# OxygenLost/dddmr_navigation

Hardware: AMD Instinct MI355X
Metric: scored trajectories/sec (N_traj x N_steps) (higher is better)
Workload: dtype f32; 1 GPU; C3: 16384 trajectories x 80 steps vs 500000-point cloud, 80-pose prune plan, shipped critic stack; scene_layout=r02, trajectories_per_gpu=16384, steps_per_trajectory=80, parallelism=single, contexts_per_gpu=1

## Files before the change

dddmr_navigation_amd/csrc/rollout_engine.hip:

```cpp
#include <hip/hip_runtime.h>
#include <dlfcn.h>
#include <rccl/rccl.h>

#include <algorithm>
#include <atomic>
#include <cmath>
#include <cstdarg>
#include <chrono>
#include <cstdio>
#include <cstdlib>
#include <cstring>
#include <memory>
#include <mutex>
#include <string>
#include <vector>

#include "rollout_kernels.hip.h"
#include "tick_plan.hip.h"
#include "perception_kernels.hip.h"
#include "depth_feed.hip.h"
#include "depth_image.hip.h"
#include "depth_clear.hip.h"
#include "lidar_sweep.hip.h"
#include "lidar_features.hip.h"
// ... 6 lines not shown

constexpr int kCloudBufs = 3;

struct MarkingState;
struct DepthMarkState;
struct DepthLayerState;
struct StackState;
struct MclState;
template <class T>
using ModuleSlot = std::unique_ptr<T, LateDelete<T>>;

struct SourceOwned {
  std::unique_ptr<PerceptionScratch> feed;
  std::unique_ptr<DepthSource> depth;
  std::unique_ptr<DepthImage> dimg;
  std::unique_ptr<LidarSweep> sweep;
  Owned scan_obs;
  float4* obs = nullptr;
  DcFrustum frustum{};
};

}

struct dddmr_rollout_ctx {
  dddmr_rollout_config cfg{};
  std::vector<dddmr_theory_config> theories;
  int device = 0;
  hipStream_t stream = nullptr, copy_stream = nullptr;
  DevAllocs mem;
  HostAllocs host;
  TrajInfo* traj_info = nullptr;
  double2* st_sc = nullptr;
  float2* st_xy = nullptr;
  size_t st_cap = 0;
  hipEvent_t ev0 = nullptr, ev1 = nullptr, evs0 = nullptr, evs1 = nullptr, cloud_ready[kCloudBufs] = {nullptr, nullptr, nullptr};

  float4* cloud_dev[kCloudBufs] = {nullptr, nullptr, nullptr};
  uint32_t cloud_n[kCloudBufs] = {0, 0, 0};
  SourceLayout cloud_layout[kCloudBufs];
  uint2* pt_slot = nullptr;
  Pt3* sorted = nullptr;
  uint32_t *cell_count = nullptr, *cell_start = nullptr;
  uint32_t* row_tab = nullptr;
  float* axes_dev = nullptr;
  float4* samples_dev = nullptr;
  float4* plan_dev = nullptr;
  float* plan_pairs_dev = nullptr;
  double* costs = nullptr;
  TrajPartial* partial = nullptr;
  int32_t* steps = nullptr;
  float4* samples_out = nullptr;
  int64_t* best_key = nullptr;
  uint32_t* overflow = nullptr;
  DevResult* result_dev = nullptr;
  uint32_t* tickets = nullptr;
  float4* blocked_plan = nullptr;
  uint32_t* blocked_flags = nullptr;
  uint32_t* traj_load = nullptr;
  uint32_t* assign = nullptr;
  TickFeedback feedback;
  TickKnobs knobs;
  bool poison = false;
  bool host_prof = false;
  bool debug_grid = false;
  int ceil_blocks = 0;
  double prof_ns[4] = {0, 0, 0, 0};
// ... 492 lines not shown

void set_no_winner(dddmr_rollout_result* out) {
  out->planner_state = DDDMR_ALL_TRAJECTORIES_FAIL;
  out->best_index = -1;
  out->best_cost = -1.0;
  out->vx = out->vy = out->wz = 0.0;
}

void no_winner(dddmr_rollout_result* out) {
  std::memset(out, 0, sizeof(*out));
  set_no_winner(out);
  out->key = kKeyNone;
}

int tick_enqueue(dddmr_rollout_ctx* ctx, const char* theory_name, const dddmr_tick_input* in) {
  const auto prof_t0 = std::chrono::steady_clock::now();
  const dddmr_theory_config* th = find_theory(ctx, theory_name);
  if (!th) return fail(ctx, DDDMR_ERR_UNKNOWN_THEORY, "unknown theory '%s'", theory_name);
  HIPCHK(ctx, hipSetDevice(ctx->device));
  Window& w = ctx->pend.window;
  make_window(*th, *in, w);

  CloudPin pin(ctx);
  Drain drain{ctx->stream, false};

  TickPlan& p = ctx->pend.plan;
  DevTick& k = p.k;
  const int theory_id = (int)(th - ctx->theories.data());
  const bool exchange = ctx->comm || ctx->comm_loopback;
  std::string err;
  const int rc = plan_tick(ctx->knobs, ctx->feedback, ctx->cfg, *th, theory_id, *in, w, pin.n_points(), ctx->plan_m,
                           ctx->plan_last, exchange, &p, &err);
  if (rc != DDDMR_OK) return fail(ctx, rc, "%s", err.c_str());
  if (ctx->seq == 3 && ctx->debug_grid)
    std::fprintf(stderr, "[dddmr] k_score shape: %d lanes, tile %d, %d-step rows, %zu bytes of dynamic LDS (tile+1 would need %zu)\n", p.thr, k.tile,
                 p.s_tick, p.score_lds, plan_score_lds(k, k.tile + 1));

  if (p.upload == kUploadList) {
    std::memcpy(ctx->small_stage, w.list.data(), w.list.size() * sizeof(float4));
    HIPCHK(ctx, hipMemcpyAsync(ctx->samples_dev, ctx->small_stage, w.list.size() * sizeof(float4), hipMemcpyHostToDevice, ctx->stream));
  } else if (p.upload == kUploadAxesDev) {
    float* a = ctx->small_stage;
    std::memcpy(a, w.ax.data(), w.ax.size() * sizeof(float));
    std::memcpy(a + k.ay_ofs, w.ay.data(), w.ay.size() * sizeof(float));
    std::memcpy(a + k.ath_ofs, w.ath.data(), w.ath.size() * sizeof(float));
    HIPCHK(ctx, hipMemcpyAsync(ctx->axes_dev, a, 3 * kMaxAxis * sizeof(float), hipMemcpyHostToDevice, ctx->stream));
  }
  if (k.n_local > 0) {
    const size_t need = (size_t)k.n_local * (size_t)p.s_tick;
    if (need > ctx->st_cap || !ctx->traj_info) {
      HIPCHK(ctx, hipDeviceSynchronize());
      ctx->st_cap = 0;
      const size_t cap = need + need / 4 + 1024;
      HIPCHK(ctx, dev_realloc(ctx->mem, &ctx->st_sc, cap));
      HIPCHK(ctx, dev_realloc(ctx->mem, &ctx->st_xy, cap));
      ctx->st_cap = cap;
      if (!ctx->traj_info) HIPCHK(ctx, dev_alloc(ctx->mem, &ctx->traj_info, (size_t)ctx->cfg.max_trajectories));
    }
  }
  HIPCHK(ctx, pin.wait_on(ctx->stream));

  const auto prof_t1 = std::chrono::steady_clock::now();
  if (ctx->poison && k.n_local > 0) {
    HIPCHK(ctx, hipMemsetAsync(ctx->costs, 0xFF, (size_t)k.n_local * sizeof(double), ctx->stream));
    HIPCHK(ctx, hipMemsetAsync(ctx->steps, 0xFF, (size_t)k.n_local * sizeof(int32_t), ctx->stream));
    HIPCHK(ctx, hipMemsetAsync(ctx->samples_out, 0xFF, (size_t)k.n_local * sizeof(float4), ctx->stream));
    HIPCHK(ctx, hipMemsetAsync(ctx->partial, 0xFF, (size_t)k.n_local * sizeof(TrajPartial), ctx->stream));
  }
  k.seq = ++ctx->seq;
  if (k.seq == 0) k.seq = ctx->seq = 1;
  const bool timed = ctx->timing >= 1 && (ctx->seq % (uint32_t)ctx->timing_every) == 0;
  const bool timed_all = timed && ctx->timing >= 2;
  if (timed_all) HIPCHK(ctx, hipEventRecord(ctx->ev0, ctx->stream));
  ctx->feedback.load_theory = theory_id;
  ctx->feedback.load_nlocal = k.n_local;
  ctx->last_heading_rows = p.heading_rows;
  ctx->last_fused_walk = k.n_local > 0 ? p.fused_walk : 0;
  drain.armed = true;
  if (k.n_points > 0) {
    hipLaunchKernelGGL(k_bin_count, dim3(p.cnt_blocks + p.roll_blocks + (k.use_assign ? k.assign_groups : 0)), dim3(kBinThreads),
                       p.roll_launch_lds, ctx->stream, k, pin.dev(), ctx->cell_count, ctx->cell_start, ctx->pt_slot, ctx->tickets,
                       ctx->best_key, ctx->overflow, ctx->axes_dev, ctx->samples_dev, ctx->traj_info, ctx->st_sc,
                       ctx->st_xy, ctx->traj_load, ctx->assign, p.heading_rows);
    hipLaunchKernelGGL(k_bin_scatter, dim3(p.bin_blocks), dim3(256), 0, ctx->stream, k, pin.dev(),
                       ctx->pt_slot, ctx->cell_start, ctx->sorted, ctx->row_tab);
  } else {
    hipLaunchKernelGGL(k_bin_reset, dim3(1), dim3(256), 0, ctx->stream, k, ctx->cell_count, ctx->cell_start,
                       ctx->best_key, ctx->overflow);
    if (p.roll_blocks > 0)
      hipLaunchKernelGGL(k_rollout, dim3(p.roll_blocks), dim3(256), p.roll_launch_lds, ctx->stream, k, ctx->axes_dev,
                         ctx->samples_dev, ctx->traj_info, ctx->st_sc, ctx->st_xy, p.heading_rows);
    if (k.use_assign)
      hipLaunchKernelGGL(k_assign, dim3(k.assign_groups), dim3(kBinThreads), 0, ctx->stream, k, ctx->traj_load, ctx->assign);
  }
  if (timed) HIPCHK(ctx, hipEventRecord(ctx->evs0, ctx->stream));
  DevResult* score_result = exchange ? ctx->local_result_dev : ctx->result_dev;
  int64_t* score_words = exchange ? ctx->slots_dev + 2 * p.rank : nullptr;
  if (k.n_local > 0) {
    const int wgs = k.n_tiles;
    const size_t lds = p.score_lds;
#define DDDMR_LAUNCH_SCORE(T, L)                                                                                   \
  do { if (k.probe) DDDMR_LAUNCH_SCORE_P(T, L, true); else DDDMR_LAUNCH_SCORE_P(T, L, false); } while (0)
#define DDDMR_LAUNCH_SCORE_P(T, L, P)                                                                              \
  hipLaunchKernelGGL((k_score<T, L, P>), dim3(wgs), dim3(T), lds, ctx->stream, k, ctx->traj_info, ctx->st_sc,     \
                     ctx->st_xy, ctx->plan_dev, ctx->cell_start, ctx->sorted, ctx->costs, ctx->steps,             \
                     ctx->samples_out, ctx->best_key, ctx->overflow, ctx->tickets + 1, score_result, ctx->assign, \
                     ctx->traj_load, score_words, ctx->row_tab, ctx->plan_pairs_dev, ctx->partial, p.fused_walk)
    if (p.thr == 512) { if (p.lean) DDDMR_LAUNCH_SCORE(512, true); else DDDMR_LAUNCH_SCORE(512, false); }
    else              { if (p.lean) DDDMR_LAUNCH_SCORE(256, true); else DDDMR_LAUNCH_SCORE(256, false); }
#undef DDDMR_LAUNCH_SCORE
#undef DDDMR_LAUNCH_SCORE_P
  } else {
    hipLaunchKernelGGL(k_empty_result, dim3(1), dim3(64), 0, ctx->stream, k, ctx->cell_start, score_result, score_words);
  }
  if (timed) HIPCHK(ctx, hipEventRecord(ctx->evs1, ctx->stream));
  if (k.n_local > 0 && k.final_kernel)
    hipLaunchKernelGGL(k_finalize, dim3((k.n_local + kFinalThreads - 1) / kFinalThreads), dim3(kFinalThreads), 0, ctx->stream, k,
                       ctx->traj_info, ctx->partial, ctx->costs, ctx->steps, ctx->samples_out, ctx->traj_load, ctx->best_key,
                       ctx->cell_start, ctx->overflow, ctx->tickets + 1, score_result, score_words);
  if (exchange) {
    if (ctx->comm) {
      const int nrc = rccl().all_reduce(ctx->slots_dev, ctx->slots_red, (size_t)2 * ctx->comm_ranks, ncclInt64, ncclMin,
                                        ctx->comm, ctx->stream);
      if (nrc != ncclSuccess) return fail(ctx, DDDMR_ERR_HIP, "ncclAllReduce failed: %s", rccl().error_string((ncclResult_t)nrc));
    } else {
      HIPCHK(ctx, hipMemcpyAsync(ctx->slots_red, ctx->slots_dev, (size_t)2 * ctx->comm_ranks * sizeof(int64_t),
                                 hipMemcpyDeviceToDevice, ctx->stream));
    }
    hipLaunchKernelGGL(k_resolve, dim3(1), dim3(64), 0, ctx->stream, k, ctx->slots_red, ctx->comm_ranks,
                       ctx->local_result_dev, ctx->axes_dev, ctx->samples_dev, ctx->result_dev);
  }
  if (timed_all) HIPCHK(ctx, hipEventRecord(ctx->ev1, ctx->stream));
  HIPCHK(ctx, hipGetLastError());
  if (ctx->host_prof) {
    const auto prof_t2 = std::chrono::steady_clock::now();
    ctx->prof_ns[0] += std::chrono::duration<double, std::nano>(prof_t1 - prof_t0).count();
    ctx->prof_ns[1] += std::chrono::duration<double, std::nano>(prof_t2 - prof_t1).count();
    ++ctx->prof_n;
  }
  pin.keep();
// ... 303 lines not shown
```

dddmr_navigation_amd/csrc/rollout_kernels.hip.h:

```cpp
#pragma once
#include <hip/hip_runtime.h>
#include <limits.h>
#include <stdint.h>

#include "../../include/dddmr_rollout.h"

#pragma clang fp contract(off)

namespace dddmr {

#ifndef DDDMR_PSPLIT_MAX
#define DDDMR_PSPLIT_MAX 4
#endif
#ifndef DDDMR_SCORE_WPE
#define DDDMR_SCORE_WPE 2
#endif
#ifndef DDDMR_SCORE_WPE_256
#define DDDMR_SCORE_WPE_256 5
#endif
#ifdef DDDMR_HANDOFF_ACQREL
#define DDDMR_HANDOFF_ORDER __ATOMIC_ACQ_REL
#else
#define DDDMR_HANDOFF_ORDER __ATOMIC_RELAXED
#endif
// ... 333 lines not shown
  } while (0)
#define DDDMR_STAMP_RAW(i)                                                                     \
  do {                                                                                         \
    if ((threadIdx.x & 63) == 0 && threadIdx.x == 0 && blockIdx.x < 16384)                       \
      g_stamps[blockIdx.x * kStampSlots + (i)] = __builtin_amdgcn_s_memtime();                   \
  } while (0)
__device__ unsigned long long g_rstamps[4096 * 8];
#define DDDMR_RSTAMP(i)                                                                        \
  do {                                                                                         \
    if (threadIdx.x == 0 && blockIdx.x < 4096) {                                                 \
      g_rstamps[blockIdx.x * 8 + (i)] = __builtin_amdgcn_s_memtime();                            \
      if ((i) == 0) g_rstamps[blockIdx.x * 8 + 4] = __builtin_amdgcn_s_memrealtime();            \
      if ((i) == 3) g_rstamps[blockIdx.x * 8 + 5] = __builtin_amdgcn_s_memrealtime();            \
    }                                                                                            \
  } while (0)
#else
#define DDDMR_STAMP(i) do { } while (0)
#define DDDMR_STAMP_RAW(i) do { } while (0)
#define DDDMR_RSTAMP(i) do { } while (0)
#endif

struct TrajInfo {
  float vx, vy, w;
  int steps;
  double dt;
  int over;
  int hrow;
};

__host__ __device__ inline size_t rollout_lds_bytes(int rt, int max_steps) {
  return (size_t)rt * (size_t)(max_steps + 1) * 16 + 16;
}

template <int kThreads>
__device__ __forceinline__ void rollout_block(const DevTick& k, const int block, const float* __restrict__ axes,
                                              const float4* __restrict__ samples, TrajInfo* __restrict__ info,
                                              double2* __restrict__ st_sc, float2* __restrict__ st_xy,
                                              unsigned char* roll_lds, const bool shared) {
  const int S1 = k.max_steps + 1;
  const int rt = k.rt;
  double2* inc = reinterpret_cast<double2*>(roll_lds);
  __shared__ int steps_s[kRolloutMax];
  __shared__ float vel_s[kRolloutMax][3];
  __shared__ double dt_s[kRolloutMax];
  __shared__ int li_s[kRolloutMax];
  __shared__ unsigned char lc_s[kRolloutMax];
  const int tid = threadIdx.x;
  const int l0 = block * rt;
  const int nt = min(rt, k.n_local - l0);
  const bool omni = (k.kind == DDDMR_THEORY_OMNI_SIMPLE);
  double2* hrow = reinterpret_cast<double2*>(roll_lds + rollout_lds_bytes(rt, k.max_steps));
  double2* qrow = hrow + 2 * S1;
  const int ns_row = k.fixed_steps <= k.max_steps ? k.fixed_steps : 0;
  int c0 = 0, ncls = 0;
  bool owns_row0 = false;
  if (shared) {
    const ClassPos first = class_major_position(k.begin, k.n_local, k.nth, l0);
    c0 = first.cls;
    owns_row0 = first.member == 0;
    ncls = class_major_position(k.begin, k.n_local, k.nth, l0 + nt - 1).cls - c0 + 1;
  }
  DDDMR_RSTAMP(0);

  if (tid < nt) {
    int li = l0 + tid, lc = 0;
    bool heads_row = false;
    if (shared) {
      const ClassPos cp = class_major_position(k.begin, k.n_local, k.nth, l0 + tid);
      li = cp.li;
      lc = cp.cls - c0;
      heads_row = tid == 0 || cp.member == 0;
// ... 123 lines not shown
          double ix = (double)fmul(vx, cf), iy = (double)fmul(vx, sf);
          if (omni) {
            const double2 q = qrow[r];
            ix += (double)vy * q.x;
            iy += (double)vy * q.y;
          }
          inc[idx] = make_double2(ix * dt_s[j], iy * dt_s[j]);
        }
      }
    }
  }
  for (int idx = tid; !shared && idx < nt * S1; idx += kThreads) {
    const int j = bj, s = bs;
    bj += stride_j;
    bs += stride_s;
    if (bs >= S1) { bs -= S1; ++bj; }
    const int ns = steps_s[j];
    if (s <= ns) {
      const double ang = (double)reinterpret_cast<const float*>(inc + idx)[(j >> 4) & 3];
      double sn, cs;
      sincos_heading(ang, &sn, &cs);
      if (s >= 1) st_sc[(size_t)(l0 + j) * k.max_steps + (s - 1)] = make_double2(cs, sn);
      if (s < ns) {
        const float vx = vel_s[j][0], vy = vel_s[j][1];
        const float cf = (float)cs, sf = (float)sn;
        double ix = (double)fmul(vx, cf), iy = (double)fmul(vx, sf);
        if (omni) {
          double s2, c2;
          sincos_quarter_ahead(ang, sn, cs, &s2, &c2);
          ix += (double)vy * c2;
          iy += (double)vy * s2;
        }
        inc[idx] = make_double2(ix * dt_s[j], iy * dt_s[j]);
      }
    }
  }
  __syncthreads();
  DDDMR_RSTAMP(2);

  static_assert(kThreads >= 2 * kRolloutMax, "phase C needs a lane per chain");
  {
    const int cj = tid & (kRolloutMax - 1), comp = tid >> 7;
    if (tid < 2 * kRolloutMax && cj < nt) {
      const int ns = steps_s[cj];
      double* ir = reinterpret_cast<double*>(inc + (size_t)cj * S1) + comp;
      float p = 0.f;
      int s = 0;
      for (; s + 4 <= ns; s += 4) {
        const double i0 = ir[2 * s], i1 = ir[2 * s + 2], i2 = ir[2 * s + 4], i3 = ir[2 * s + 6];
        p = (float)((double)p + i0); *reinterpret_cast<float*>(ir + 2 * s) = p;
        p = (float)((double)p + i1); *reinterpret_cast<float*>(ir + 2 * s + 2) = p;
        p = (float)((double)p + i2); *reinterpret_cast<float*>(ir + 2 * s + 4) = p;
        p = (float)((double)p + i3); *reinterpret_cast<float*>(ir + 2 * s + 6) = p;
      }
      for (; s < ns; ++s) {
        p = (float)((double)p + ir[2 * s]);
        *reinterpret_cast<float*>(ir + 2 * s) = p;
      }
    }
  }
  __syncthreads();
  bj = tid / S1;
  bs = tid - bj * S1;
  for (int idx = tid; idx < nt * S1; idx += kThreads) {
    const int j = bj, s = bs;
    bj += stride_j;
    bs += stride_s;
    if (bs >= S1) { bs -= S1; ++bj; }
    if (s < steps_s[j]) {
      const float* slot = reinterpret_cast<const float*>(inc + idx);
      st_xy[(size_t)li_s[j] * k.max_steps + s] = make_float2(slot[0], slot[2]);
    }
  }
  DDDMR_RSTAMP(3);
}

__device__ __forceinline__ int tile_round_base(const DevTick& k, int r) {
  return r < k.r0 ? r * k.nb_tiles : k.r0 * k.nb_tiles + (r - k.r0) * k.n_tiles;
}
__device__ __forceinline__ int tile_slot(const DevTick& k, int b, int j) {
  return tile_round_base(k, b < k.nb_tiles ? j : j + k.r0) + b;
}
constexpr int kAssignPer = 4;
template <int kThreads>
__device__ __forceinline__ void assign_block(const DevTick& k, const int grp, const uint32_t* __restrict__ load,
                                             uint32_t* __restrict__ assign) {
  __shared__ uint32_t hist[kLoadClasses];
  __shared__ uint32_t wsum[kThreads / 64];
  __shared__ uint32_t mx_s, mn_s;
  static_assert(kLoadClasses == kThreads, "one class per lane in the scan");
  const int tid = threadIdx.x;
  const int G = k.assign_groups;
  const int n = k.n_local, tl = k.n_tiles / G, tlb = k.nb_tiles / G;
  const int ng = (n - grp + G - 1) / G;
  auto group_slot = [&](int r) {
    const int early = k.r0 * tlb;
    int start, width, round;
    if (r < early) { round = r / tlb; start = round * tlb; width = tlb; }
    else { round = k.r0 + (r - early) / tl; start = early + (round - k.r0) * tl; width = tl; }
    const int pos = r - start;
    const int bl = ((round & 1) && start + width <= ng) ? width - 1 - pos : pos;
    return grp + G * (start + bl);
  };
  DDDMR_RSTAMP(0);
  hist[tid] = 0;
// ... 27 lines not shown
  for (int e = 0; e < kAssignPer; ++e) {
    const int m = tid + e * kThreads;
    if (m < ng) atomicAdd(&hist[kLoadClasses - 1 - min(kLoadClasses - 1, (int)((float)v[e] * scale))], 1u);
  }
  __syncthreads();
  const uint32_t cnt = hist[tid];
  const uint32_t inc = wave_incl_scan_u32(cnt);
  if ((tid & 63) == 63) wsum[tid >> 6] = inc;
  __syncthreads();
  uint32_t base = inc - cnt;
  for (int w = 0; w < (tid >> 6); ++w) base += wsum[w];
  hist[tid] = base;
  __syncthreads();
#pragma unroll
  for (int e = 0; e < kAssignPer; ++e) {
    const int m = tid + e * kThreads;
    if (m < ng) {
      const int c = kLoadClasses - 1 - min(kLoadClasses - 1, (int)((float)v[e] * scale));
      const int r = (int)atomicAdd(&hist[c], 1u);
      assign[group_slot(r)] = (uint32_t)(grp + G * m);
    }
  }
  DDDMR_RSTAMP(3);
}

__global__ __launch_bounds__(kBinThreads) void k_assign(DevTick k, const uint32_t* __restrict__ load,
                                                        uint32_t* __restrict__ assign) {
  assign_block<kBinThreads>(k, (int)blockIdx.x, load, assign);
}

__global__ __launch_bounds__(256) void k_rollout(DevTick k, const float* __restrict__ axes,
                                                 const float4* __restrict__ samples,
                                                 TrajInfo* __restrict__ info, double2* __restrict__ st_sc,
                                                 float2* __restrict__ st_xy, const int heading_rows) {
  extern __shared__ __attribute__((aligned(16))) unsigned char dyn_lds[];
  rollout_block<256>(k, (int)blockIdx.x, axes, samples, info, st_sc, st_xy, dyn_lds, heading_rows != 0);
}

__global__ __launch_bounds__(kBinThreads, 8) void k_bin_count(DevTick k, const float4* __restrict__ cloud,
                                                   uint32_t* __restrict__ cell_count,
                                                   uint32_t* __restrict__ cell_start,
                                                   uint2* __restrict__ pt_slot, uint32_t* __restrict__ ticket,
                                                   int64_t* __restrict__ best_key,
                                                   uint32_t* __restrict__ overflow, const float* __restrict__ axes,
                                                   const float4* __restrict__ samples, TrajInfo* __restrict__ info,
                                                   double2* __restrict__ st_sc, float2* __restrict__ st_xy,
                                                   const uint32_t* __restrict__ load, uint32_t* __restrict__ assign,
                                                   const int heading_rows) {
  extern __shared__ __attribute__((aligned(16))) unsigned char dyn_lds[];
  const int n_assign = k.use_assign ? k.assign_groups : 0;
  if ((int)blockIdx.x < n_assign) {
    assign_block<kBinThreads>(k, (int)blockIdx.x, load, assign);
    return;
  }
  if ((int)blockIdx.x < n_assign + k.roll_blocks) {
    rollout_block<kBinThreads>(k, (int)blockIdx.x - n_assign, axes, samples, info, st_sc, st_xy, dyn_lds, heading_rows != 0);
    return;
  }
  const int bin_block = (int)blockIdx.x - n_assign - k.roll_blocks;
  __shared__ uint32_t wave_sum[16];
  __shared__ uint32_t carry_s;
  __shared__ uint32_t is_last;
  const int stride = k.bin_blocks * blockDim.x;
  DDDMR_RSTAMP(0);
  for (int base = bin_block * blockDim.x + threadIdx.x; base < k.n_points; base += stride * kBinPer) {
    float4 p[kBinPer];
    uint2 slot[kBinPer];
#pragma unroll
    for (int m = 0; m < kBinPer; ++m) {
      const int i = base + m * stride;
      p[m] = i < k.n_points ? cloud[i] : make_float4(0.f, 0.f, 0.f, 0.f);
    }
#pragma unroll
    for (int m = 0; m < kBinPer; ++m) {
      const int i = base + m * stride;
      slot[m] = make_uint2(0xFFFFFFFFu, 0u);
      const bool in = i < k.n_points && p[m].x >= k.rmin[0] && p[m].x <= k.rmax[0] && p[m].y >= k.rmin[1] &&
                      p[m].y <= k.rmax[1] && p[m].z >= k.rmin[2] && p[m].z <= k.rmax[2];
      if (in) {
        const int c = cell_of(k, p[m].x, p[m].y, p[m].z);
        slot[m].x = (uint32_t)c;
        slot[m].y = atomicAdd(&cell_count[c], 1u);
      }
    }
#pragma unroll
    for (int m = 0; m < kBinPer; ++m) {
      const int i = base + m * stride;
      if (i < k.n_points) pt_slot[i] = slot[m];
    }
// ... 202 lines not shown
    }
    if (r < 0) { cost = r; done = true; }
    else cost += r;
  }
  *cbits = cost_bits(cost);
  return cost;
}

__host__ __device__ inline uint32_t traj_load_of(int plan_m, int walked, int steps, bool collided) {
  return (uint32_t)walked + (uint32_t)steps * (2u + (collided ? 0u : (uint32_t)((plan_m + 15) >> 4)));
}

__device__ __forceinline__ f2 dot3_2(f2 dx, f2 dy, f2 dz, float a, float b, float c) {
#pragma clang fp contract(off)
  return (dx * a + dy * b) + dz * c;
}
__device__ __forceinline__ int box_test2(const float* r, const Pt3 a, const Pt3 b, bool use_radius) {
#pragma clang fp contract(off)
  const f2 x = {a.x, b.x}, y = {a.y, b.y}, z = {a.z, b.z};
  const f2 dx = x - r[0], dy = y - r[1], dz = z - r[2];
  const f2 xv = __builtin_elementwise_abs(dot3_2(dx, dy, dz, r[3], r[4], r[5]));
  const f2 yv = __builtin_elementwise_abs(dot3_2(dx, dy, dz, r[6], r[7], r[8]));
  const f2 zv = __builtin_elementwise_abs(dot3_2(dx, dy, dz, r[9], r[10], r[11]));
  bool h0 = xv.x <= r[12] && yv.x <= r[13] && zv.x <= r[14];
  bool h1 = xv.y <= r[12] && yv.y <= r[13] && zv.y <= r[14];
  if (use_radius) {
    const f2 d2 = l2_simple2(x, y, z, r[15], r[16], r[17]);
    h0 = h0 && d2.x < 1.0f;
    h1 = h1 && d2.y < 1.0f;
  }
  return (h0 ? 1 : 0) | (h1 ? 2 : 0);
}

__device__ __forceinline__ void pose_translation(const DevTick& k, float2 bxy, double T[3]) {
#pragma unroll
  for (int i = 0; i < 3; ++i) T[i] = k.R[3 * i + 0] * (double)bxy.x + k.R[3 * i + 1] * (double)bxy.y + k.t[i];
}

__device__ __forceinline__ void obb_axes_in_place(float* r) {
  float v[4][3];
#pragma unroll
  for (int a = 0; a < 4; ++a) { v[a][0] = r[3 + 3 * a]; v[a][1] = r[4 + 3 * a]; v[a][2] = r[5 + 3 * a]; }
  const int vi[3] = {3, 1, 2};
#pragma unroll
  for (int a = 0; a < 3; ++a) {
    const float ex = fsub(v[vi[a]][0], v[0][0]), ey = fsub(v[vi[a]][1], v[0][1]), ez = fsub(v[vi[a]][2], v[0][2]);
    const float len = sqrtf(dot3(ex, ey, ez, ex, ey, ez));
    r[12 + a] = len * 0.5f;
    r[3 + 3 * a + 0] = ex / len;
    r[3 + 3 * a + 1] = ey / len;
    r[3 + 3 * a + 2] = ez / len;
  }
}

template <bool kStamps>
__device__ __forceinline__ void reduce_slots(const DevTick& k, const int lane, const int n_slots,
                                             const unsigned long long* __restrict__ slots,
                                             const uint32_t* __restrict__ cell_start, const uint32_t* __restrict__ overflow,
                                             DevResult* __restrict__ result, int64_t* __restrict__ words_out) {
  constexpr int kPer = 8;
  const uint32_t n_binned = cell_start[k.n_cells];
  const uint32_t over = __hip_atomic_load(overflow, __ATOMIC_RELAXED, __HIP_MEMORY_SCOPE_AGENT);
  long long bc = (long long)kKeyNone;
  long long bi = -1;
  unsigned long long b2 = 0, b3 = 0;
  uint32_t n_coll = 0;
  for (int base = 0; base < n_slots; base += 64 * kPer) {
    unsigned long long w[kPer][kSlotWords];
#pragma unroll
    for (int u = 0; u < kPer; ++u) {
      const int i = base + u * 64 + lane;
// ... 34 lines not shown
    r.n_collided = n_coll;
    if (kStamps) DDDMR_STAMP_RAW(17);
    *result = r;
    if (words_out) {
      words_out[0] = any ? (int64_t)bc : kKeyNone;
      words_out[1] = any ? -(int64_t)r.index : kKeyNone;
    } else {
      __threadfence_system();
      __hip_atomic_store(&result->seq, k.seq, __ATOMIC_RELEASE, __HIP_MEMORY_SCOPE_SYSTEM);
    }
    if (kStamps) DDDMR_STAMP_RAW(18);
  }
}

__device__ __forceinline__ double stick_sum_wave(const float* dr, const int ns, const int lane) {
  double acc = 0.0;
  for (int s2 = lane; s2 < ns; s2 += 64) acc += (double)dr[s2];
  acc += dpp_row_shl<8>(acc);
  acc += dpp_row_shl<4>(acc);
  acc += dpp_row_shl<2>(acc);
  acc += dpp_row_shl<1>(acc);
  const double r1 = __shfl(acc, 16, 64), r2 = __shfl(acc, 32, 64), r3 = __shfl(acc, 48, 64);
  return (acc + r1) + (r2 + r3);
}

template <int kScoreThreads, bool kLean, bool kProbe>
__global__ __launch_bounds__(kScoreThreads, kScoreThreads >= 512 ? DDDMR_SCORE_WPE : DDDMR_SCORE_WPE_256) void k_score(
    DevTick k, const TrajInfo* __restrict__ info, const double2* __restrict__ st_sc, const float2* __restrict__ st_xy,
    const float4* __restrict__ plan_xyz, const uint32_t* __restrict__ cell_start,
    const Pt3* __restrict__ sorted, double* __restrict__ costs, int32_t* __restrict__ steps_out,
    float4* __restrict__ samples_out, int64_t* __restrict__ best_key, uint32_t* __restrict__ overflow,
    uint32_t* __restrict__ ticket, DevResult* __restrict__ result, const uint32_t* __restrict__ assign,
    uint32_t* __restrict__ traj_load, int64_t* __restrict__ words_out, const uint32_t* __restrict__ row_tab,
    const float* __restrict__ plan_pairs, TrajPartial* __restrict__ partial, const int fused_walk) {
  extern __shared__ __attribute__((aligned(16))) unsigned char lds_raw[];
  const int tile = k.tile;
  const int S1 = k.max_steps + 1;
  const int Qcap = tile * k.max_steps;
  constexpr bool kCanFuse = kLean && kScoreThreads == 512;
  const bool fused = kCanFuse && fused_walk != 0 && Qcap <= kScoreThreads && k.m > 0 && k.want_collision != 0 && k.n_points >= 5;
  const bool need_box = k.want_collision != 0, need_mm = !kLean && k.want_minmax != 0;
  const bool rec_pose = !kLean && k.rec_pose != 0;
  const bool box_fast = kLean || k.box_fast != 0;
  const int rec_words = rec_words_of(rec_pose, need_mm);
  const int mm_ofs = kRecBase + (rec_pose ? 3 : 0);
  size_t ofs = 0;
  TrajHead* head = reinterpret_cast<TrajHead*>(lds_raw);
  ofs += sizeof(TrajHead) * (size_t)tile;
  ofs = (ofs + 15) & ~(size_t)15;
  float4* plan = reinterpret_cast<float4*>(lds_raw + ofs);
  ofs += 16 * (size_t)(k.m > 0 ? k.m : 1);
  float4* ppos = reinterpret_cast<float4*>(lds_raw + ofs);
  ofs += 16 * (size_t)Qcap;
  float* dist = reinterpret_cast<float*>(lds_raw + ofs);
  ofs += 4 * (size_t)tile * S1;
  float* rec = reinterpret_cast<float*>(lds_raw + ofs);
  ofs += 4 * (size_t)rec_words * Qcap;
  uint32_t* tab = reinterpret_cast<uint32_t*>(lds_raw + ofs);
  ofs += 4 * (size_t)k.tab_entries;
  ofs = (ofs + 15) & ~(size_t)15;
  uint32_t* pref = reinterpret_cast<uint32_t*>(lds_raw + ofs);
  uint32_t* seg_p = pref + ((size_t)Qcap * k.rows_cap + 1);
  uint32_t* seg_len = seg_p + (size_t)Qcap * k.rows_cap;
  ofs += 4 * ((size_t)Qcap * k.rows_cap + 1) + 8 * ((size_t)Qcap * k.rows_cap) + 16;
  ofs = (ofs + 7) & ~(size_t)7;
  unsigned long long* wsum64 = reinterpret_cast<unsigned long long*>(lds_raw + ofs);

  __shared__ int alive_pairs_s;
  __shared__ uint32_t t_item0[kMaxTile + 1];
  __shared__ uint32_t t_ubase[kMaxTile + 1];
  const int tid = threadIdx.x;
  const int lane = tid & 63, wid = tid >> 6;
  const int tb = (int)blockIdx.x;
  int nt = 0;
  for (int j = 0; j < tile; ++j) nt += ((tb < k.nb_tiles || j + k.r0 < tile) && tile_slot(k, tb, j) < k.n_local) ? 1 : 0;

  DDDMR_STAMP(0);
  for (int i = tid; i < k.m; i += kScoreThreads) plan[i] = plan_xyz[i];

  if (tid < nt) {
    const int slot = tile_slot(k, tb, tid);
    const int li = k.use_assign ? (int)assign[slot] : slot;
    const TrajInfo ti = info[li];
    if (ti.over) atomicOr(overflow, 1u);
    TrajHead h;
    h.vx = ti.vx; h.vy = ti.vy; h.w = ti.w;
    h.steps = ti.steps;
    h.dt = ti.dt;
    h.pair_base = 0;
    h.hit_box = 0; h.hit_mm = 0; h.aux = ti.hrow;
    h.pp_dist = 0.0; h.pp_yaw = 0.0; h.stick_sum = 0.0;
    h.li = li;
    h.walked = 0;
    head[tid] = h;
  }
  const int tab_n = k.tab_entries;
  const bool tab_staged = tab_n > 0;
  if (tab_staged && k.n_points >= 5 && (need_box || need_mm)) {
    for (int i = tid; i < tab_n; i += kScoreThreads) tab[i] = row_tab[i];
  }
  __syncthreads();
  DDDMR_STAMP(1);
  if (tid < 64) {
    const uint32_t st = tid < nt ? (uint32_t)head[tid].steps : 0u;
    const uint32_t incl = wave_incl_scan_u32(st);
    if (tid < nt) head[tid].pair_base = (int)(incl - st);
  }
  __syncthreads();
  DDDMR_STAMP(2);
  DDDMR_STAMP(3);
  int total_pairs = 0;
  if (nt > 0) total_pairs = head[nt - 1].pair_base + head[nt - 1].steps;
  const bool cloud_ok = k.n_points >= 5;
  const bool do_coll = cloud_ok && (need_box || need_mm);
  for (int q = tid; q < total_pairs; q += kScoreThreads) {
    int j = 0;
    while (j + 1 < nt && head[j + 1].pair_base <= q) ++j;
    const int s = q - head[j].pair_base;
    const size_t so = (size_t)head[j].li * k.max_steps + s;
    const double2 cs = st_sc[(size_t)head[j].aux * k.max_steps + s];
    const float2 bxy = st_xy[so];
    const double c = cs.x, sn = cs.y;
    double L[9], T[3];
#pragma unroll
    for (int i = 0; i < 3; ++i) {
      const double r0 = k.R[3 * i + 0], r1 = k.R[3 * i + 1], r2 = k.R[3 * i + 2];
      L[3 * i + 0] = r0 * c + r1 * sn;
      L[3 * i + 1] = r1 * c - r0 * sn;
      L[3 * i + 2] = r2;
    }
    pose_translation(k, bxy, T);
    const float px = (float)T[0], py = (float)T[1], pz = (float)T[2];
    ppos[q] = make_float4(px, py, pz, kCanFuse ? __int_as_float(j * S1 + s) : 0.f);

    if (do_coll) {
      float v[4][3];
      float mnx = 3.402823466e+38f, mny = mnx, mnz = mnx, mxx = -mnx, mxy = -mnx, mxz = -mnx;
      float ccx = 0.f, ccy = 0.f, ccz = 0.f;
      float vmax2 = 0.f;
      auto world_vertex = [&](int vtx, float& wx, float& wy, float& wz) {
        const double cx = k.cub[3 * vtx + 0], cy = k.cub[3 * vtx + 1], cz = k.cub[3 * vtx + 2];
        wx = (float)(L[0] * cx + L[1] * cy + L[2] * cz + T[0]);
        wy = (float)(L[3] * cx + L[4] * cy + L[5] * cz + T[1]);
        wz = (float)(L[6] * cx + L[7] * cy + L[8] * cz + T[2]);
        mnx = fminf(mnx, wx); mxx = fmaxf(mxx, wx);
        mny = fminf(mny, wy); mxy = fmaxf(mxy, wy);
        mnz = fminf(mnz, wz); mxz = fmaxf(mxz, wz);
        ccx = fadd(ccx, wx); ccy = fadd(ccy, wy); ccz = fadd(ccz, wz);
        if (rec_pose) {
          const float ux = wx - px, uy = wy - py, uz = wz - pz;
          vmax2 = fmaxf(vmax2, ux * ux + uy * uy + uz * uz);
        }
      };
      if (box_fast && !rec_pose) {
        const double X0 = k.cub[0], X1 = k.cub[9], Y0 = k.cub[1], Y1 = k.cub[4], Z0 = k.cub[2], Z1 = k.cub[8];
// ... 55 lines not shown
          if (rec_pose) far_corner(c1x * s1, c1y * s1, c1z * s1, c2x * s2, c2y * s2, c2z * s2, c3x * s3, c3y * s3, c3z * s3);
        }
        obx = obx * 1.00001f + 1e-4f;
        oby = oby * 1.00001f + 1e-4f;
      }
      float* r = rec + (size_t)q * rec_words;
      r[0] = ccx / 8.f; r[1] = ccy / 8.f; r[2] = ccz / 8.f;
#pragma unroll
      for (int a = 0; a < 4; ++a) {
        r[3 + 3 * a + 0] = v[a][0];
        r[3 + 3 * a + 1] = v[a][1];
        r[3 + 3 * a + 2] = v[a][2];
      }
      const float gx = k.gmin[0], gy = k.gmin[1];
      const float ocx = ccx / 8.f - gx, ocy = ccy / 8.f - gy, prx = px - gx, pry = py - gy;
      const float lox = fmaxf(fminf(mnx - gx, ocx - obx), prx - 1.0f), hix = fminf(fmaxf(mxx - gx, ocx + obx), prx + 1.0f);
      const float loy = fmaxf(fminf(mny - gy, ocy - oby), pry - 1.0f), hiy = fminf(fmaxf(mxy - gy, ocy + oby), pry + 1.0f);
      int cx0 = (int)floorf(lox * k.inv_cell), cx1 = (int)floorf(hix * k.inv_cell);
      int cy0 = (int)floorf(loy * k.inv_cell), cy1 = (int)floorf(hiy * k.inv_cell);
      cx0 = max(cx0, 0); cy0 = max(cy0, 0);
      cx1 = min(cx1, k.gnx - 1); cy1 = min(cy1, k.gny - 1);
      if (cx0 > cx1 || cy0 > cy1) { cx0 = 1; cx1 = 0; cy0 = 1; cy1 = 0; }
      reinterpret_cast<int*>(r)[15] = (cx0 & 0xFFFF) | (cx1 << 16);
      reinterpret_cast<int*>(r)[16] = (cy0 & 0xFFFF) | (cy1 << 16);
      reinterpret_cast<int*>(r)[17] = j | ((vmax2 < 0.99f || !rec_pose) ? 0x10000 : 0);
      if (rec_pose) { r[18] = px; r[19] = py; r[20] = pz; }
      if (need_mm) {
        float* rm = r + mm_ofs;
        rm[0] = mnx; rm[1] = mny; rm[2] = mnz; rm[3] = mxx; rm[4] = mxy; rm[5] = mxz;
      }
      if (cy1 - cy0 + 1 > k.rows_cap) atomicOr(overflow, 2u);
    }
  }
  if (tid < nt && head[tid].steps > 0) {
    const int j = tid;
    const size_t so = (size_t)head[j].li * k.max_steps + (head[j].steps - 1);
    const double2 cs = st_sc[(size_t)head[j].aux * k.max_steps + (head[j].steps - 1)];
    const float2 bxy = st_xy[so];
    const double c = cs.x, sn = cs.y;
    double L[9], T[3];
#pragma unroll
    for (int i = 0; i < 3; ++i) {
      const double r0 = k.R[3 * i + 0], r1 = k.R[3 * i + 1], r2 = k.R[3 * i + 2];
      L[3 * i + 0] = r0 * c + r1 * sn;
      L[3 * i + 1] = r1 * c - r0 * sn;
      L[3 * i + 2] = r2;
    }
    pose_translation(k, bxy, T);
    const double d0 = k.planT[0] - T[0], d1 = k.planT[1] - T[1], d2 = k.planT[2] - T[2];
    const double tx = L[0] * d0 + L[3] * d1 + L[6] * d2;
    const double ty = L[1] * d0 + L[4] * d1 + L[7] * d2;
    const double tz = L[2] * d0 + L[5] * d1 + L[8] * d2;
    const double D00 = L[0] * k.planR[0] + L[3] * k.planR[3] + L[6] * k.planR[6];
    const double D10 = L[1] * k.planR[0] + L[4] * k.planR[3] + L[7] * k.planR[6];
    const double D20 = L[2] * k.planR[0] + L[5] * k.planR[3] + L[8] * k.planR[6];
    double yaw = 0.0;
    if (fabs(D20) < 1.0) yaw = atan2(D10, D00);
    head[j].pp_dist = sqrt(tx * tx + ty * ty + tz * tz);
    head[j].pp_yaw = fmod(yaw + 3.1416, 3.1416);
  }
  __syncthreads();

  DDDMR_STAMP(4);
  if (do_coll && total_pairs > 0) {
    unsigned long long carry = 0;
    if (tid <= kMaxTile) t_item0[tid] = 0u;
    for (int base = 0; base < total_pairs; base += kScoreThreads) {
      const int q = base + tid;
      uint32_t rb[kRows], rl[kRows];
#pragma unroll
      for (int r = 0; r < kRows; ++r) { rb[r] = 0; rl[r] = 0; }
      unsigned long long cnt = 0;
      if (q < total_pairs) {
        const int* ri = reinterpret_cast<const int*>(rec + (size_t)q * rec_words);
        const int cx0 = (short)(ri[15] & 0xFFFF), cx1 = ri[15] >> 16;
        const int cy0 = (short)(ri[16] & 0xFFFF), cy1 = ri[16] >> 16;
        if (cx0 <= cx1) {
#pragma unroll
          for (int r = 0; r < kRows; ++r) {
            const int cy = cy0 + r;
            if (cy <= cy1) {
              uint32_t b, e;
              if (tab_staged) {
                b = tab[cy * (k.gnx + 1) + cx0];
                e = tab[cy * (k.gnx + 1) + cx1 + 1];
              } else {
                b = cell_start[(cy * k.gnx + cx0) * k.gnz];
                e = cell_start[(cy * k.gnx + cx1 + 1) * k.gnz];
              }
              rb[r] = b;
              rl[r] = e - b;
              if (e > b) cnt += (1ull << 32) | (unsigned long long)((e - b + kItem - 1) / kItem);
            }
// ... 75 lines not shown
      r[15] = r[16] = r[17] = 0.f;
      if (use_radius || need_mm) { r[15] = rq[18]; r[16] = rq[19]; r[17] = rq[20]; }
      bool fb = false, fm = false;
      if (need_box) {
        int hits = 0;
  #pragma unroll
        for (int u = 0; u < kItem; u += 2) {
          const int h2 = box_test2(r, pt[u], pt[u + 1], use_radius);
          hits |= h2 << u;
        }
        fb = (hits & ((1 << n) - 1)) != 0;
      }
      if (need_mm) {
  #pragma unroll
        for (int u = 0; u < kItem; ++u) {
          const bool in = (uint32_t)u < n && l2_simple(r[15], r[16], r[17], pt[u].x, pt[u].y, pt[u].z) < 1.0f;
          const float* rm = rq + mm_ofs;
          fm |= in && (pt[u].x >= rm[0] && pt[u].x <= rm[3] && pt[u].y >= rm[1] && pt[u].y <= rm[4] &&
                       pt[u].z >= rm[2] && pt[u].z <= rm[5]);
        }
      }
      if (fb) atomicOr(&head[j].hit_box, 1);
      if (fm) atomicOr(&head[j].hit_mm, 1);
    };
    auto find_seg = [&](uint32_t item, int lo) {
      int hi = nseg;
      while (hi - lo > 1) {
        const int mid = (lo + hi) >> 1;
        if (pref[mid] <= item) lo = mid; else hi = mid;
      }
      return lo;
    };
    const int n_rounds = (kProbe && total > (uint32_t)kScoreThreads) ? 2 : 1;
    for (int round = 0; round < n_rounds; ++round) {
      if (tid < 64) {
        uint32_t cnt = 0;
        if (tid < nt) {
          const bool decided = round > 0 && (!need_box || head[tid].hit_box != 0) && (!need_mm || head[tid].hit_mm != 0);
          if (!decided) cnt = t_item0[tid + 1] - t_item0[tid];
        }
        const uint32_t incl = wave_incl_scan_u32(cnt);
        if (tid < nt) t_ubase[tid] = incl - cnt;
        if (tid == nt - 1) t_ubase[nt] = incl;
      }
      __syncthreads();
      const uint32_t tot_r = t_ubase[nt];
      const uint32_t chunk = (tot_r + kScoreThreads - 1) / kScoreThreads;
      uint32_t p = (uint32_t)tid * chunk;
      const uint32_t p1 = min(tot_r, p + ((round == 0 && n_rounds == 2) ? 1u : chunk));
      if (p < p1) {
        int j = 0;
        while (t_ubase[j + 1] <= p) ++j;
        uint32_t it = t_item0[j] + (p - t_ubase[j]);
        int sg = find_seg(it, 0);
        for (;;) {
          walk_item(it, sg);
          if (++p >= p1) break;
          if (p >= t_ubase[j + 1]) {
            do { ++j; } while (t_ubase[j + 1] <= p);
            it = t_item0[j] + (p - t_ubase[j]);
            sg = find_seg(it, sg);
          } else {
            ++it;
            while (pref[sg + 1] <= it) ++sg;
          }
        }
      }
      if (!(fused && round + 1 == n_rounds)) __syncthreads();
    }
    if (fused) {
      const bool mine = tid < total_pairs;
      float px = 0.f, py = 0.f, pz = 0.f, best = 3.402823466e+38f;
      int dst = 0;
      if (mine) {
        const float4 pp = ppos[tid];
        px = pp.x; py = pp.y; pz = pp.z;
        dst = __float_as_int(pp.w);
      }
      if (__ballot(mine) != 0ull) {
        constexpr uint32_t kPoseBytes = 4u * kPlanPoseWords, kChunkBytes = kPoseBytes * kPlanChunk;
        const uint32_t end = kPoseBytes * (uint32_t)k.m;
        PlanChunk ca = plan_request(plan_pairs, 0u);
        plan_wait(ca, best);
        for (uint32_t o = 0; o < end; o += 2u * kChunkBytes) {
          PlanChunk cb = plan_request(plan_pairs, o + kChunkBytes);
          plan_current(ca);
          best = plan_chunk_min(best, ca, px, py, pz);
          plan_wait(cb, best);
          ca = plan_request(plan_pairs, o + 2u * kChunkBytes);
          plan_current(cb);
          best = plan_chunk_min(best, cb, px, py, pz);
          plan_wait(ca, best);
        }
// ... 416 lines not shown
```

Baseline: 123.4 million trajectories/s.

## Move pure-pursuit pose into rollout, prefetch score staging, skip single-round scan

```diff
diff --git a/dddmr_navigation_amd/csrc/rollout_engine.hip b/dddmr_navigation_amd/csrc/rollout_engine.hip
--- a/dddmr_navigation_amd/csrc/rollout_engine.hip
+++ b/dddmr_navigation_amd/csrc/rollout_engine.hip
@@ -62,6 +62,7 @@
   TrajInfo* traj_info = nullptr;
   double2* st_sc = nullptr;
   float2* st_xy = nullptr;
+  double2* st_pp = nullptr;
   size_t st_cap = 0;
   hipEvent_t ev0 = nullptr, ev1 = nullptr, evs0 = nullptr, evs1 = nullptr, cloud_ready[kCloudBufs] = {nullptr, nullptr, nullptr};
 
@@ -620,6 +621,8 @@
   const int rc = plan_tick(ctx->knobs, ctx->feedback, ctx->cfg, *th, theory_id, *in, w, pin.n_points(), ctx->plan_m,
                            ctx->plan_last, exchange, &p, &err);
   if (rc != DDDMR_OK) return fail(ctx, rc, "%s", err.c_str());
+  if (ctx->seq == 0 && ctx->debug_grid)
+    std::fprintf(stderr, "[dddmr] grid: %d x %d x %d cells, row-run index of %d entries in LDS\n", k.gnx, k.gny, k.gnz, k.tab_entries);
   if (ctx->seq == 3 && ctx->debug_grid)
     std::fprintf(stderr, "[dddmr] k_score shape: %d lanes, tile %d, %d-step rows, %zu bytes of dynamic LDS (tile+1 would need %zu)\n", p.thr, k.tile,
                  p.s_tick, p.score_lds, plan_score_lds(k, k.tile + 1));
@@ -642,6 +645,7 @@
       const size_t cap = need + need / 4 + 1024;
       HIPCHK(ctx, dev_realloc(ctx->mem, &ctx->st_sc, cap));
       HIPCHK(ctx, dev_realloc(ctx->mem, &ctx->st_xy, cap));
+      HIPCHK(ctx, dev_realloc(ctx->mem, &ctx->st_pp, (size_t)ctx->cfg.max_trajectories));
       ctx->st_cap = cap;
       if (!ctx->traj_info) HIPCHK(ctx, dev_alloc(ctx->mem, &ctx->traj_info, (size_t)ctx->cfg.max_trajectories));
     }
@@ -654,6 +658,7 @@
     HIPCHK(ctx, hipMemsetAsync(ctx->steps, 0xFF, (size_t)k.n_local * sizeof(int32_t), ctx->stream));
     HIPCHK(ctx, hipMemsetAsync(ctx->samples_out, 0xFF, (size_t)k.n_local * sizeof(float4), ctx->stream));
     HIPCHK(ctx, hipMemsetAsync(ctx->partial, 0xFF, (size_t)k.n_local * sizeof(TrajPartial), ctx->stream));
+    HIPCHK(ctx, hipMemsetAsync(ctx->st_pp, 0xFF, (size_t)k.n_local * sizeof(double2), ctx->stream));
   }
   k.seq = ++ctx->seq;
   if (k.seq == 0) k.seq = ctx->seq = 1;
@@ -669,7 +674,7 @@
     hipLaunchKernelGGL(k_bin_count, dim3(p.cnt_blocks + p.roll_blocks + (k.use_assign ? k.assign_groups : 0)), dim3(kBinThreads),
                        p.roll_launch_lds, ctx->stream, k, pin.dev(), ctx->cell_count, ctx->cell_start, ctx->pt_slot, ctx->tickets,
                        ctx->best_key, ctx->overflow, ctx->axes_dev, ctx->samples_dev, ctx->traj_info, ctx->st_sc,
-                       ctx->st_xy, ctx->traj_load, ctx->assign, p.heading_rows);
+                       ctx->st_xy, ctx->st_pp, ctx->traj_load, ctx->assign, p.heading_rows);
     hipLaunchKernelGGL(k_bin_scatter, dim3(p.bin_blocks), dim3(256), 0, ctx->stream, k, pin.dev(),
                        ctx->pt_slot, ctx->cell_start, ctx->sorted, ctx->row_tab);
   } else {
@@ -677,7 +682,7 @@
                        ctx->best_key, ctx->overflow);
     if (p.roll_blocks > 0)
       hipLaunchKernelGGL(k_rollout, dim3(p.roll_blocks), dim3(256), p.roll_launch_lds, ctx->stream, k, ctx->axes_dev,
-                         ctx->samples_dev, ctx->traj_info, ctx->st_sc, ctx->st_xy, p.heading_rows);
+                         ctx->samples_dev, ctx->traj_info, ctx->st_sc, ctx->st_xy, ctx->st_pp, p.heading_rows);
     if (k.use_assign)
       hipLaunchKernelGGL(k_assign, dim3(k.assign_groups), dim3(kBinThreads), 0, ctx->stream, k, ctx->traj_load, ctx->assign);
   }
@@ -693,7 +698,8 @@
   hipLaunchKernelGGL((k_score<T, L, P>), dim3(wgs), dim3(T), lds, ctx->stream, k, ctx->traj_info, ctx->st_sc,     \
                      ctx->st_xy, ctx->plan_dev, ctx->cell_start, ctx->sorted, ctx->costs, ctx->steps,             \
                      ctx->samples_out, ctx->best_key, ctx->overflow, ctx->tickets + 1, score_result, ctx->assign, \
-                     ctx->traj_load, score_words, ctx->row_tab, ctx->plan_pairs_dev, ctx->partial, p.fused_walk)
+                     ctx->traj_load, score_words, ctx->row_tab, ctx->plan_pairs_dev, ctx->partial, p.fused_walk,  \
+                     ctx->st_pp)
     if (p.thr == 512) { if (p.lean) DDDMR_LAUNCH_SCORE(512, true); else DDDMR_LAUNCH_SCORE(512, false); }
     else              { if (p.lean) DDDMR_LAUNCH_SCORE(256, true); else DDDMR_LAUNCH_SCORE(256, false); }
 #undef DDDMR_LAUNCH_SCORE
diff --git a/dddmr_navigation_amd/csrc/rollout_kernels.hip.h b/dddmr_navigation_amd/csrc/rollout_kernels.hip.h
--- a/dddmr_navigation_amd/csrc/rollout_kernels.hip.h
+++ b/dddmr_navigation_amd/csrc/rollout_kernels.hip.h
@@ -389,11 +389,39 @@
   return (size_t)rt * (size_t)(max_steps + 1) * 16 + 16;
 }
 
+__host__ __device__ __forceinline__ void pose_translation(const DevTick& k, float2 bxy, double T[3]) {
+#pragma unroll
+  for (int i = 0; i < 3; ++i) T[i] = k.R[3 * i + 0] * (double)bxy.x + k.R[3 * i + 1] * (double)bxy.y + k.t[i];
+}
+
+__host__ __device__ inline double2 pure_pursuit_last_pose(const DevTick& k, const float2 bxy, const double2 cs) {
+  const double c = cs.x, sn = cs.y;
+  double L[9], T[3];
+#pragma unroll
+  for (int i = 0; i < 3; ++i) {
+    const double r0 = k.R[3 * i + 0], r1 = k.R[3 * i + 1], r2 = k.R[3 * i + 2];
+    L[3 * i + 0] = r0 * c + r1 * sn;
+    L[3 * i + 1] = r1 * c - r0 * sn;
+    L[3 * i + 2] = r2;
+  }
+  pose_translation(k, bxy, T);
+  const double d0 = k.planT[0] - T[0], d1 = k.planT[1] - T[1], d2 = k.planT[2] - T[2];
+  const double tx = L[0] * d0 + L[3] * d1 + L[6] * d2;
+  const double ty = L[1] * d0 + L[4] * d1 + L[7] * d2;
+  const double tz = L[2] * d0 + L[5] * d1 + L[8] * d2;
+  const double D00 = L[0] * k.planR[0] + L[3] * k.planR[3] + L[6] * k.planR[6];
+  const double D10 = L[1] * k.planR[0] + L[4] * k.planR[3] + L[7] * k.planR[6];
+  const double D20 = L[2] * k.planR[0] + L[5] * k.planR[3] + L[8] * k.planR[6];
+  double yaw = 0.0;
+  if (fabs(D20) < 1.0) yaw = atan2(D10, D00);
+  return make_double2(sqrt(tx * tx + ty * ty + tz * tz), fmod(yaw + 3.1416, 3.1416));
+}
+
 template <int kThreads>
 __device__ __forceinline__ void rollout_block(const DevTick& k, const int block, const float* __restrict__ axes,
                                               const float4* __restrict__ samples, TrajInfo* __restrict__ info,
                                               double2* __restrict__ st_sc, float2* __restrict__ st_xy,
-                                              unsigned char* roll_lds, const bool shared) {
+                                              double2* __restrict__ st_pp, unsigned char* roll_lds, const bool shared) {
   const int S1 = k.max_steps + 1;
   const int rt = k.rt;
   double2* inc = reinterpret_cast<double2*>(roll_lds);
@@ -583,6 +611,8 @@
           iy += (double)vy * s2;
         }
         inc[idx] = make_double2(ix * dt_s[j], iy * dt_s[j]);
+      } else if (s >= 1) {
+        inc[idx] = make_double2(cs, sn);
       }
     }
   }
@@ -622,6 +652,16 @@
       const float* slot = reinterpret_cast<const float*>(inc + idx);
       st_xy[(size_t)li_s[j] * k.max_steps + s] = make_float2(slot[0], slot[2]);
     }
+  }
+  if (tid < nt) {
+    const int ns = steps_s[tid];
+    double2 pp = make_double2(0.0, 0.0);
+    if (ns > 0) {
+      const float* slot = reinterpret_cast<const float*>(inc + (size_t)tid * S1 + (ns - 1));
+      const double2 cs = shared ? hrow[(int)lc_s[tid] * S1 + ns] : inc[(size_t)tid * S1 + ns];
+      pp = pure_pursuit_last_pose(k, make_float2(slot[0], slot[2]), cs);
+    }
+    st_pp[li_s[tid]] = pp;
   }
   DDDMR_RSTAMP(3);
 }
@@ -715,9 +755,10 @@
 __global__ __launch_bounds__(256) void k_rollout(DevTick k, const float* __restrict__ axes,
                                                  const float4* __restrict__ samples,
                                                  TrajInfo* __restrict__ info, double2* __restrict__ st_sc,
-                                                 float2* __restrict__ st_xy, const int heading_rows) {
+                                                 float2* __restrict__ st_xy, double2* __restrict__ st_pp,
+                                                 const int heading_rows) {
   extern __shared__ __attribute__((aligned(16))) unsigned char dyn_lds[];
-  rollout_block<256>(k, (int)blockIdx.x, axes, samples, info, st_sc, st_xy, dyn_lds, heading_rows != 0);
+  rollout_block<256>(k, (int)blockIdx.x, axes, samples, info, st_sc, st_xy, st_pp, dyn_lds, heading_rows != 0);
 }
 
 __global__ __launch_bounds__(kBinThreads, 8) void k_bin_count(DevTick k, const float4* __restrict__ cloud,
@@ -728,8 +769,8 @@
                                                    uint32_t* __restrict__ overflow, const float* __restrict__ axes,
                                                    const float4* __restrict__ samples, TrajInfo* __restrict__ info,
                                                    double2* __restrict__ st_sc, float2* __restrict__ st_xy,
-                                                   const uint32_t* __restrict__ load, uint32_t* __restrict__ assign,
-                                                   const int heading_rows) {
+                                                   double2* __restrict__ st_pp, const uint32_t* __restrict__ load,
+                                                   uint32_t* __restrict__ assign, const int heading_rows) {
   extern __shared__ __attribute__((aligned(16))) unsigned char dyn_lds[];
   const int n_assign = k.use_assign ? k.assign_groups : 0;
   if ((int)blockIdx.x < n_assign) {
@@ -737,7 +778,7 @@
     return;
   }
   if ((int)blockIdx.x < n_assign + k.roll_blocks) {
-    rollout_block<kBinThreads>(k, (int)blockIdx.x - n_assign, axes, samples, info, st_sc, st_xy, dyn_lds, heading_rows != 0);
+    rollout_block<kBinThreads>(k, (int)blockIdx.x - n_assign, axes, samples, info, st_sc, st_xy, st_pp, dyn_lds, heading_rows != 0);
     return;
   }
   const int bin_block = (int)blockIdx.x - n_assign - k.roll_blocks;
@@ -1006,11 +1047,6 @@
   return (h0 ? 1 : 0) | (h1 ? 2 : 0);
 }
 
-__device__ __forceinline__ void pose_translation(const DevTick& k, float2 bxy, double T[3]) {
-#pragma unroll
-  for (int i = 0; i < 3; ++i) T[i] = k.R[3 * i + 0] * (double)bxy.x + k.R[3 * i + 1] * (double)bxy.y + k.t[i];
-}
-
 __device__ __forceinline__ void obb_axes_in_place(float* r) {
   float v[4][3];
 #pragma unroll
@@ -1111,7 +1147,8 @@
     float4* __restrict__ samples_out, int64_t* __restrict__ best_key, uint32_t* __restrict__ overflow,
     uint32_t* __restrict__ ticket, DevResult* __restrict__ result, const uint32_t* __restrict__ assign,
     uint32_t* __restrict__ traj_load, int64_t* __restrict__ words_out, const uint32_t* __restrict__ row_tab,
-    const float* __restrict__ plan_pairs, TrajPartial* __restrict__ partial, const int fused_walk) {
+    const float* __restrict__ plan_pairs, TrajPartial* __restrict__ partial, const int fused_walk,
+    const double2* __restrict__ st_pp) {
   extern __shared__ __attribute__((aligned(16))) unsigned char lds_raw[];
   const int tile = k.tile;
   const int S1 = k.max_steps + 1;
@@ -1155,12 +1192,35 @@
   for (int j = 0; j < tile; ++j) nt += ((tb < k.nb_tiles || j + k.r0 < tile) && tile_slot(k, tb, j) < k.n_local) ? 1 : 0;
 
   DDDMR_STAMP(0);
-  for (int i = tid; i < k.m; i += kScoreThreads) plan[i] = plan_xyz[i];
-
-  if (tid < nt) {
+  const bool has_traj = tid < nt;
+  int li = 0;
+  if (has_traj) {
     const int slot = tile_slot(k, tb, tid);
-    const int li = k.use_assign ? (int)assign[slot] : slot;
+    li = k.use_assign ? (int)assign[slot] : slot;
+  }
+  const int tab_n = k.tab_entries;
+  const bool tab_staged = tab_n > 0;
+  const bool copy_tab = tab_staged && k.n_points >= 5 && (need_box || need_mm);
+  constexpr int kTabQuads = kTabCap / (4 * kScoreThreads);
+  static_assert(kTabQuads * 4 * kScoreThreads == kTabCap, "the index copy covers kTabCap exactly");
+  const int tab_q = tab_n >> 2, tab_r = tab_n & 3;
+  uint4 tq[kTabQuads];
+  uint32_t tq_tail = 0u;
+  if (copy_tab) {
+    const int last_q = tab_q > 0 ? tab_q - 1 : 0;
+#pragma unroll
+    for (int e = 0; e < kTabQuads; ++e) {
+      tq[e] = make_uint4(0u, 0u, 0u, 0u);
+      if (tab_q > 0) tq[e] = reinterpret_cast<const uint4*>(row_tab)[min(tid + e * kScoreThreads, last_q)];
+    }
+    if (tid < tab_r) tq_tail = row_tab[4 * tab_q + tid];
+  }
+  const bool copy_plan = !fused;
+  float4 plan_mine = make_float4(0.f, 0.f, 0.f, 0.f);
+  if (copy_plan && tid < k.m) plan_mine = plan_xyz[tid];
+  if (has_traj) {
     const TrajInfo ti = info[li];
+    const double2 pp = st_pp[li];
     if (ti.over) atomicOr(overflow, 1u);
     TrajHead h;
     h.vx = ti.vx; h.vy = ti.vy; h.w = ti.w;
@@ -1168,15 +1228,24 @@
     h.dt = ti.dt;
     h.pair_base = 0;
     h.hit_box = 0; h.hit_mm = 0; h.aux = ti.hrow;
-    h.pp_dist = 0.0; h.pp_yaw = 0.0; h.stick_sum = 0.0;
+    h.pp_dist = pp.x; h.pp_yaw = pp.y; h.stick_sum = 0.0;
     h.li = li;
     h.walked = 0;
     head[tid] = h;
   }
-  const int tab_n = k.tab_entries;
-  const bool tab_staged = tab_n > 0;
-  if (tab_staged && k.n_points >= 5 && (need_box || need_mm)) {
-    for (int i = tid; i < tab_n; i += kScoreThreads) tab[i] = row_tab[i];
+  if (copy_tab) {
+#pragma unroll
+    for (int e = 0; e < kTabQuads; ++e) {
+      const int i4 = tid + e * kScoreThreads;
+      if (i4 < tab_q) {
+        tab[4 * i4 + 0] = tq[e].x; tab[4 * i4 + 1] = tq[e].y; tab[4 * i4 + 2] = tq[e].z; tab[4 * i4 + 3] = tq[e].w;
+      }
+    }
+    if (tid < tab_r) tab[4 * tab_q + tid] = tq_tail;
+  }
+  if (copy_plan) {
+    if (tid < k.m) plan[tid] = plan_mine;
+    for (int i = tid + kScoreThreads; i < k.m; i += kScoreThreads) plan[i] = plan_xyz[i];
   }
   __syncthreads();
   DDDMR_STAMP(1);
@@ -1198,8 +1267,9 @@
     const int s = q - head[j].pair_base;
     const size_t so = (size_t)head[j].li * k.max_steps + s;
     const double2 cs = st_sc[(size_t)head[j].aux * k.max_steps + s];
-    const float2 bxy = st_xy[so];
-    const double c = cs.x, sn = cs.y;
+    float2 bxy = st_xy[so];
+    double c = cs.x, sn = cs.y;
+    asm volatile("" : "+v"(c), "+v"(sn), "+v"(bxy.x), "+v"(bxy.y));
     double L[9], T[3];
 #pragma unroll
     for (int i = 0; i < 3; ++i) {
@@ -1321,33 +1391,7 @@
       if (cy1 - cy0 + 1 > k.rows_cap) atomicOr(overflow, 2u);
     }
   }
-  if (tid < nt && head[tid].steps > 0) {
-    const int j = tid;
-    const size_t so = (size_t)head[j].li * k.max_steps + (head[j].steps - 1);
-    const double2 cs = st_sc[(size_t)head[j].aux * k.max_steps + (head[j].steps - 1)];
-    const float2 bxy = st_xy[so];
-    const double c = cs.x, sn = cs.y;
-    double L[9], T[3];
-#pragma unroll
-    for (int i = 0; i < 3; ++i) {
-      const double r0 = k.R[3 * i + 0], r1 = k.R[3 * i + 1], r2 = k.R[3 * i + 2];
-      L[3 * i + 0] = r0 * c + r1 * sn;
-      L[3 * i + 1] = r1 * c - r0 * sn;
-      L[3 * i + 2] = r2;
-    }
-    pose_translation(k, bxy, T);
-    const double d0 = k.planT[0] - T[0], d1 = k.planT[1] - T[1], d2 = k.planT[2] - T[2];
-    const double tx = L[0] * d0 + L[3] * d1 + L[6] * d2;
-    const double ty = L[1] * d0 + L[4] * d1 + L[7] * d2;
-    const double tz = L[2] * d0 + L[5] * d1 + L[8] * d2;
-    const double D00 = L[0] * k.planR[0] + L[3] * k.planR[3] + L[6] * k.planR[6];
-    const double D10 = L[1] * k.planR[0] + L[4] * k.planR[3] + L[7] * k.planR[6];
-    const double D20 = L[2] * k.planR[0] + L[5] * k.planR[3] + L[8] * k.planR[6];
-    double yaw = 0.0;
-    if (fabs(D20) < 1.0) yaw = atan2(D10, D00);
-    head[j].pp_dist = sqrt(tx * tx + ty * ty + tz * tz);
-    head[j].pp_yaw = fmod(yaw + 3.1416, 3.1416);
-  }
+  DDDMR_STAMP(19);
   __syncthreads();
 
   DDDMR_STAMP(4);
@@ -1489,7 +1533,9 @@
       return lo;
     };
     const int n_rounds = (kProbe && total > (uint32_t)kScoreThreads) ? 2 : 1;
+    const uint32_t* const t_ubase_r = n_rounds == 1 ? t_item0 : t_ubase;
     for (int round = 0; round < n_rounds; ++round) {
+      if (n_rounds > 1) {
       if (tid < 64) {
         uint32_t cnt = 0;
         if (tid < nt) {
@@ -1501,21 +1547,22 @@
         if (tid == nt - 1) t_ubase[nt] = incl;
       }
       __syncthreads();
-      const uint32_t tot_r = t_ubase[nt];
+      }
+      const uint32_t tot_r = t_ubase_r[nt];
       const uint32_t chunk = (tot_r + kScoreThreads - 1) / kScoreThreads;
       uint32_t p = (uint32_t)tid * chunk;
       const uint32_t p1 = min(tot_r, p + ((round == 0 && n_rounds == 2) ? 1u : chunk));
       if (p < p1) {
         int j = 0;
-        while (t_ubase[j + 1] <= p) ++j;
-        uint32_t it = t_item0[j] + (p - t_ubase[j]);
+        while (t_ubase_r[j + 1] <= p) ++j;
+        uint32_t it = t_item0[j] + (p - t_ubase_r[j]);
         int sg = find_seg(it, 0);
         for (;;) {
           walk_item(it, sg);
           if (++p >= p1) break;
-          if (p >= t_ubase[j + 1]) {
-            do { ++j; } while (t_ubase[j + 1] <= p);
-            it = t_item0[j] + (p - t_ubase[j]);
+          if (p >= t_ubase_r[j + 1]) {
+            do { ++j; } while (t_ubase_r[j + 1] <= p);
+            it = t_item0[j] + (p - t_ubase_r[j]);
             sg = find_seg(it, sg);
           } else {
             ++it;
```

Result: faster. 127.5 million trajectories/s (median of 6 runs) (+3.4%).
